# jthorborg/signalizer

Hardware: AMD Instinct MI355X
Metric: 32768-pt stereo STFT frames/sec (75% overlap); achieved HBM GB/s vs peak (higher is better)
Workload: dtype f32

## Files before the change

signalizer_amd/csrc/api.hip:

```cpp
#include <hip/hip_runtime.h>

#include <algorithm>
#include <chrono>
#include <cmath>
#include <atomic>
#include <cstdlib>
#include <cstring>
#include <deque>
#include <mutex>
#include <new>
#include <string>
#include <vector>

#include "runtime.hpp"
#include "trace.hpp"

namespace sgz {

thread_local std::string g_lastError;
#ifdef SGZ_SCHED_SWEEP
int g_schedule[7] = {-1, -1, -1, -1, -1, -1, -1};
#endif
#ifdef SGZ_DEBUG
uint32_t g_ablate = 0;
// ... 163 lines not shown
sgz_status resetResonator(Plan &p, hipStream_t stream)
{
    if (!isResonator(p) || !p.d_resState) return SGZ_OK;
    SGZ_HIP(hipMemsetAsync(p.d_resState, 0, size_t(p.C) * 2 * size_t(p.resV) * p.P * 2 * sizeof(float), stream));
    return SGZ_OK;
}

static sgz_status fillResParams(Plan &p, const float *d_planar, size_t chStride, long frames, float *d_mapped, uint32_t hopOverride, ResParams &r)
{
    r = ResParams{};
    r.planar = d_planar; r.chStride = chStride; r.frames = frames;
    r.hop = hopOverride ? hopOverride : p.cfg.hop; r.C = p.C; r.P = p.P; r.mode = p.cfg.channel_mode;
    r.V = p.resV; r.signals = p.stateChannels; r.sides = p.sides; r.firstContinues = true;
    r.coeff = reinterpret_cast<const float2 *>(p.d_resCoeff);
    r.cpow = reinterpret_cast<const float4 *>(p.d_resPow);
    r.cpowB = reinterpret_cast<const float2 *>(p.d_resPowB);
    r.cpowBLo = reinterpret_cast<const float2 *>(p.d_resPowBLo);
    r.matrixForm = p.optMatrixResonator;
    r.w1 = p.optMatrixResonator ? reinterpret_cast<const float2 *>(p.d_resW1) : nullptr;
    r.w2 = reinterpret_cast<const float2 *>(p.d_resW2);
    r.w1b = reinterpret_cast<const uint4 *>(p.d_resW1b);
    r.tilePow = reinterpret_cast<const float4 *>(p.d_resTile);
    r.gain = p.d_resGain;
    for (int v = 0; v < 9; ++v) r.weights[v] = p.resWeights[v];
    r.state = reinterpret_cast<float2 *>(p.d_resState);
    const size_t perFrame = size_t(p.C) * size_t(r.signals) * size_t(r.V) * p.P;
    sgz_status st = ensureCap(&p.d_resLocal, &p.resLocalCap, (size_t(frames) + size_t(kResSegments)) * perFrame * 2);
    if (st != SGZ_OK) return st;
    r.local = reinterpret_cast<float2 *>(p.d_resLocal);
    r.segEnd = r.local + size_t(frames) * perFrame;
    r.mapped = d_mapped;
    return SGZ_OK;
}

static sgz_status runResonator(Plan &p, const float *d_planar, size_t chStride, long frames, float *d_mapped, hipStream_t stream, uint32_t hopOverride = 0,
                               bool skipWindow = false)
{
    if (frames <= 0) return SGZ_OK;
    if (!d_mapped) return fail(SGZ_EUNSUPPORTED, "the resonator algorithm has no transform bins: ask for mapped values");
    if (hopOverride && frames != 1) return fail(SGZ_EINVAL, "a block advance of the resonators is one frame");
    if (!skipWindow && !hopOverride) {
        const size_t perFrame = size_t(p.C) * size_t(p.stateChannels) * size_t(p.resV) * p.P * 2 * sizeof(float);
        const long slab = p.optResonatorSlab ? long(p.optResonatorSlab) : long(std::max<size_t>(64, (size_t(256) << 20) / perFrame));
        if (frames > slab) {
            for (long f0 = 0; f0 < frames; f0 += slab) {
                const long nf = std::min(slab, frames - f0);
                const sgz_status st = runResonator(p, d_planar + size_t(f0) * p.cfg.hop, chStride, nf, d_mapped + size_t(f0) * p.C * p.sides * p.P, stream);
                if (st != SGZ_OK) return st;
            }
            return SGZ_OK;
        }
    }
    ResParams r;
    if (sgz_status st = fillResParams(p, d_planar, chStride, frames, d_mapped, hopOverride, r); st != SGZ_OK) return st;
    r.skipWindow = skipWindow;
    SGZ_HIP(launchResonator(r, stream));
    return SGZ_OK;
}

sgz_status checkResonatorShardBound(const Plan &p, long frames)
{
    const size_t perFrame = size_t(p.C) * size_t(p.stateChannels) * size_t(p.resV) * p.P * 2 * sizeof(float);
    const size_t bound = p.optResonatorShardBound ? size_t(p.optResonatorShardBound) : std::max<size_t>(64, (size_t(8) << 30) / std::max<size_t>(perFrame, 1));
    if (frames > 0 && size_t(frames) > bound)
        return fail(SGZ_EUNSUPPORTED, "sharded RSNT render: a rank's chunk of " + std::to_string(frames) + " frames holds " +
                                          std::to_string((size_t(frames) * perFrame) >> 20) + " MiB of per-frame resonator states between the two halves of the render, above the bound of " +
                                          std::to_string(bound) + " frames (SGZ_OPT_RESONATOR_SHARD_BOUND; default 8 GiB): use more ranks or a shorter buffer per call");
    return SGZ_OK;
}
sgz_status runResonatorFromRest(Plan &p, const float *d_planar, size_t chStride, long frames, float *d_mapped, hipStream_t stream)
{
    if (sgz_status st = checkResonatorShardBound(p, frames); st != SGZ_OK) return st;
    if (sgz_status st = resetResonator(p, stream); st != SGZ_OK) return st;
    return runResonator(p, d_planar, chStride, frames, d_mapped, stream, 0, true);
}
sgz_status runResonatorJoin(Plan &p, long frames, float *d_mapped, const float *d_allEnd, const long long *framesPerRank, uint32_t world, uint32_t rank,
                            float *d_carry, hipStream_t stream)
{
    if (frames <= 0) return SGZ_OK;
    ResParams r;
    if (sgz_status st = fillResParams(p, nullptr, 0, frames, d_mapped, 0, r); st != SGZ_OK) return st;
    const float2 *carry = nullptr;
    if (rank > 0) {
        SGZ_HIP(launchResonatorFold(r, reinterpret_cast<const float2 *>(d_allEnd), framesPerRank, world, rank, reinterpret_cast<float2 *>(d_carry), stream));
        carry = reinterpret_cast<const float2 *>(d_carry);
    }
    SGZ_HIP(launchResonatorCarry(r, carry, stream));
    return SGZ_OK;
}

sgz_status runResonatorAdvance(Plan &p, const float *d_planar, size_t chStride, uint32_t nsamples, float *d_mapped, hipStream_t stream)
{
    if (!isResonator(p)) return fail(SGZ_EINVAL, "not a resonator plan");
    if (nsamples == 0) return SGZ_OK;
    return runResonator(p, d_planar, chStride, 1, d_mapped, stream, nsamples);
}

sgz_status ensureSecondStream(Plan &p)
{
    if (!p.shardStream) { hipStream_t cs; SGZ_HIP(hipStreamCreateWithFlags(&cs, hipStreamNonBlocking)); p.shardStream = cs; }
    for (void *&e : p.shardEv)
        if (!e) { hipEvent_t ne; SGZ_HIP(hipEventCreateWithFlags(&ne, hipEventDisableTiming)); e = ne; }
    return SGZ_OK;
}

sgz_status runStft(Plan &p, const float *d_planar, size_t chStride, long frames, float *d_mapped,
                          float *d_binsOut, const float *d_binsIn, hipStream_t stream, unsigned long long *d_phaseClock, bool deferLate,
                          bool imageOnly)
{
    TraceRange range("sgz::runStft (K_A)");
    p.lateDeferred = nullptr; p.lateFrames = 0;
    if (isResonator(p)) {
        if (d_binsOut || d_binsIn) return fail(SGZ_EUNSUPPORTED, "the resonator algorithm has no transform bins");
        return runResonator(p, d_planar, chStride, frames, d_mapped, stream);
    }
    const bool phase = p.cfg.channel_mode == SGZ_CH_PHASE;
    StftParams prm = fillStftParams(p, d_planar, chStride, frames, d_mapped, d_binsOut, d_binsIn, d_phaseClock);
    const long tasks = frames * long(p.C);
    if (tasks <= 0) return SGZ_OK;
    if (tasks > 0x7fffffffL) return fail(SGZ_EINVAL, "too many (frame, pair) tasks for one launch");
    if (p.optChannelSplit && ((p.realMono && d_binsIn == nullptr) || p.realSplit)) {
        const size_t units = size_t(tasks) * 2;
        if (p.nyCap < units) {
            for (float **b : {&p.d_ny, &p.d_nyBest, &p.d_low}) if (*b) { (void)hipFree(*b); *b = nullptr; }
            p.nyCap = 0;
            SGZ_HIP(hipMalloc(reinterpret_cast<void **>(&p.d_nyBest), units * 64 * sizeof(float)));
            SGZ_HIP(hipMalloc(reinterpret_cast<void **>(&p.d_ny), units * sizeof(float)));
            SGZ_HIP(hipMalloc(reinterpret_cast<void **>(&p.d_low), units * kLowBins * sizeof(float)));
            p.nyCap = units;
        }
        RealParams rp{};
        rp.planar = d_planar; rp.chStride = chStride; rp.frames = frames;
        rp.hop = p.cfg.hop; rp.C = p.C; rp.P = p.P; rp.mode = p.cfg.channel_mode;
        rp.window = p.d_windowHalf;
        rp.winPhase = p.optFetchWindow ? nullptr : reinterpret_cast<const float4 *>(p.d_winPhase); rp.winP0 = 0.5f * p.winP0; rp.winP1 = 0.5f * p.winP1;
        rp.tw1 = reinterpret_cast<const float2 *>(p.d_twReal1);
        rp.tw2 = reinterpret_cast<const float2 *>(p.d_tw2);
        rp.twPost = reinterpret_cast<const float2 *>(p.d_twRealPost);
        rp.tw2Full = reinterpret_cast<const float4 *>(p.d_tw2Full);
        rp.recs = p.d_recsReal ? p.d_recsReal : p.d_recs; rp.recsFull = p.d_recs; rp.weights = p.d_weights;
        rp.chunkEnds = p.d_chunkEnds; rp.chunkReBase = p.d_chunkReBase; rp.chunkRec = p.d_chunkRec; rp.weights12 = p.d_weights12;
        rp.chunkSlots[0] = p.chunkSlots[0]; rp.chunkSlots[1] = p.chunkSlots[1];
        rp.low = p.d_low; rp.lowPixels = p.d_realLowPixels; rp.lowCount[0] = p.realLowCount[0]; rp.lowCount[1] = p.realLowCount[1];
        rp.invSize = p.scalars.invSize;
        rp.mapped = d_mapped; rp.binsOut = d_binsOut; rp.binsIn = d_binsIn;
        rp.ny = p.d_ny; rp.nyBest = p.d_nyBest;
        rp.fixFrom[0] = p.realFixFrom[0]; rp.fixFrom[1] = p.realFixFrom[1];
        if (deferLate && !p.realMono && d_mapped && !d_binsOut && p.realLowCount[0] + p.realLowCount[1] == 0) { rp.lateInNext = 1u; p.lateDeferred = d_mapped; p.lateFrames = frames; }
        rp.roundSize = uint32_t(numCUs()) * (p.N == 16384 ? 4u : p.N == 32768 ? 2u : 1u);
        rp.pipelined = p.optPipelined ? 1u : 0u;
        if (imageOnly && rp.lateInNext && p.optImageOnlySplit && p.realSplit && p.cfg.channel_mode == SGZ_CH_SEPARATE && p.N == 32768 &&
            rp.winPhase && p.C == 1) {
            const long room = long(rp.roundSize) - tasks;
            const long want = p.optImageOnlySplit >= 2 ? long(p.optImageOnlySplit) : room > 0 ? std::min<long>(8, std::max<long>(1, (tasks + room - 1) / room)) : 4;
            rp.nyFrames = uint32_t(std::min<long>(want, frames));
        }
        p.lastNyFrames = rp.nyFrames;
        if (rp.nyFrames && !rp.pipelined && tasks > long(rp.roundSize >> 1) && tasks < long(rp.roundSize)) {
            rp.mateAdjacent = SGZ_MATE_ADJACENT;
            const long nyUnits = long(p.C) * ((frames + long(rp.nyFrames) - 1) / long(rp.nyFrames));
            if (rp.nyFrames <= 3u && tasks + nyUnits <= long(rp.roundSize)) {
                rp.prioFirst = SGZ_PRIO_FIRST; rp.prioMate = SGZ_PRIO_MATE; rp.prioNy = SGZ_PRIO_NY; rp.prioScope = SGZ_PRIO_SCOPE;
            }
#ifdef SGZ_SCHED_SWEEP
            if (g_schedule[0] >= 0) rp.nyDelay = uint32_t(g_schedule[0]);
            if (g_schedule[1] >= 0) rp.mateDelay = uint32_t(g_schedule[1]);
            if (g_schedule[2] >= 0) rp.mateAdjacent = uint32_t(g_schedule[2]);
            if (g_schedule[3] >= 0) rp.prioFirst = uint32_t(g_schedule[3]) & 3u;
            if (g_schedule[4] >= 0) rp.prioMate = uint32_t(g_schedule[4]) & 3u;
            if (g_schedule[5] >= 0) rp.prioNy = uint32_t(g_schedule[5]) & 3u;
            if (g_schedule[6] >= 0) rp.prioScope = uint32_t(g_schedule[6]) & 3u;
#endif
        }
#ifdef SGZ_DEBUG
        rp.phaseClock = d_phaseClock; rp.clkUnit = g_ablate >> 16;
#endif
        SGZ_HIP(launchStftReal(rp, p.N, stream));
        return SGZ_OK;
    }
    if (p.halves && d_binsIn == nullptr) {
        const size_t perTask = size_t(p.N) + 1;
        long slab = long(std::max<size_t>(1, (size_t(32) << 20) / perTask));
        slab = std::max<long>(1, slab / long(p.C)) * long(p.C);
        slab = std::min<long>(slab, tasks);
        if (d_binsOut == nullptr && p.binsSlab < size_t(slab)) {
            if (p.d_halfBins) { (void)hipFree(p.d_halfBins); p.d_halfBins = nullptr; }
            SGZ_HIP(hipMalloc(reinterpret_cast<void **>(&p.d_halfBins), size_t(slab) * perTask * sizeof(float)));
            p.binsSlab = size_t(slab);
        }
        if (prm.nDcPixels) { sgz_status st = ensureDcWork(p, size_t(slab)); if (st != SGZ_OK) return st; prm.dcOut = reinterpret_cast<float2 *>(p.d_dcWork); }
        for (long t0 = 0; t0 < tasks; t0 += slab) {
            const long nt = std::min(slab, tasks - t0);
            float *bins = d_binsOut ? d_binsOut + size_t(t0) * perTask : p.d_halfBins;
            prm.taskBase = t0;
            prm.frames = nt / long(p.C);
            prm.binsOut = bins;
            prm.binsSplit = (d_binsOut == nullptr && p.sideMapOk && mapSidesFit(prm, p.N)) ? 1u : 0u;
            SGZ_HIP(launchStftHalves(prm, p.N, int(2 * nt), stream));
            if (d_mapped) {
                float *out = d_mapped + size_t(t0) * p.sides * p.P;
                if (prm.binsSplit) SGZ_HIP(launchMapSides(prm, p.N, bins, nt, out, stream));
                else SGZ_HIP(launchGenericMap(prm, p.N, bins, nt, out, stream));
                SGZ_HIP(launchComplexDcFix(prm, p.N, bins, prm.dcOut, nt, out, stream));
            }
        }
        return SGZ_OK;
    }
    if (!p.fused) {
        const size_t perTask = size_t(p.N) * 2;
        long slab = long(std::max<size_t>(1, (size_t(64) << 20) / perTask));
        slab = std::max<long>(1, slab / long(p.C)) * long(p.C);
        slab = std::min<long>(slab, tasks);
        if (p.workSlab < size_t(slab)) {
            for (float **b : {&p.d_work0, &p.d_work1, &p.d_binsWork}) if (*b) { (void)hipFree(*b); *b = nullptr; }
            SGZ_HIP(hipMalloc(reinterpret_cast<void **>(&p.d_work0), size_t(slab) * perTask * sizeof(float)));
            SGZ_HIP(hipMalloc(reinterpret_cast<void **>(&p.d_work1), size_t(slab) * perTask * sizeof(float)));
            SGZ_HIP(hipMalloc(reinterpret_cast<void **>(&p.d_binsWork), size_t(slab) * (size_t(p.N) + 1) * sizeof(float) * (phase ? 2 : 1)));
            p.workSlab = size_t(slab);
        }
        if (prm.nDcPixels) { sgz_status st = ensureDcWork(p, p.workSlab); if (st != SGZ_OK) return st; prm.dcOut = reinterpret_cast<float2 *>(p.d_dcWork); }
        PhaseTables ph{};
        if (phase) {
            ph.type = p.d_phaseType; ph.norm = p.d_phaseNorm; ph.normFinal = p.phaseNormFinal;
            ph.filtered = p.cfg.bin_interp != SGZ_INTERP_NONE;
            ph.fusedFft = p.phaseFusedFft ? 1u : 0u;
            ph.csfOut = reinterpret_cast<float2 *>(d_binsOut);
            ph.csfIn = reinterpret_cast<const float2 *>(d_binsIn);
        }
        SGZ_HIP(launchGeneric(prm, p.N, reinterpret_cast<const float2 *>(p.d_twN), reinterpret_cast<float2 *>(p.d_work0),
                              reinterpret_cast<float2 *>(p.d_work1), p.d_binsWork, long(p.workSlab), stream, phase ? &ph : nullptr,
                              p.sideMapOk && !phase));
        return SGZ_OK;
    }
    const int grid = int(tasks);
    SGZ_HIP(launchStftMap(prm, p.N, grid, stream));
    return SGZ_OK;
}

static sgz_status fillDecayParams(Plan &p, const float *d_mapped, long frames, uint8_t *d_rgba, float *d_lines, float *d_state,
                                  hipStream_t stream, DecayParams &prm)
{
    prm = DecayParams{};
    prm.mapped = d_mapped;
    prm.frames = frames;
    prm.P = p.P; prm.C = p.C; prm.sides = uint32_t(p.sides);
    prm.chunk = 8;
    prm.numChunks = uint32_t((frames + prm.chunk - 1) / prm.chunk);
    prm.slope = p.d_slope;
    prm.colourTables = p.d_colourTables;
    prm.sc = p.scalars;
    prm.state = d_state; prm.stateIn = d_state; prm.rgba = d_rgba; prm.lines = d_lines;
    prm.colourOnly = (!d_state && !d_lines && d_rgba) ? 1u : 0u;
    prm.magScale = p.cfg.channel_mode == SGZ_CH_PHASE ? 0.5f : 1.0f;
    if (d_state && frames > 1) {
        const size_t stateN = size_t(p.C) * SGZ_NUM_GRAPHS * p.P * 2;
        sgz_status st0 = ensureCap(&p.d_stateCopy, &p.stateCopyCap, stateN);
        if (st0 != SGZ_OK) return st0;
        if (prm.numChunks > 1 && p.cfg.channel_mode != SGZ_CH_PHASE) {
            prm.stateStash = p.d_stateCopy;
        } else {
            SGZ_HIP(hipMemcpyAsync(p.d_stateCopy, d_state, stateN * sizeof(float), hipMemcpyDeviceToDevice, stream));
            prm.stateIn = p.d_stateCopy;
        }
    }
    return SGZ_OK;
}

sgz_status runDecayColour(Plan &p, const float *d_mapped, long frames, uint8_t *d_rgba, float *d_lines,
                                 float *d_state, hipStream_t stream, bool magnitudeOnly)
{
    TraceRange range("sgz::runDecayColour (K_B)");
    float *pending = const_cast<float *>(p.lateDeferred);
    const long pendingFrames = p.lateFrames;
    p.lateDeferred = nullptr; p.lateFrames = 0;
    if (frames <= 0) return SGZ_OK;
    p.aggMapped = nullptr;
    DecayParams prm;
    sgz_status stp = fillDecayParams(p, d_mapped, frames, d_rgba, d_lines, d_state, stream, prm);
    if (stp != SGZ_OK) return stp;
    const bool noFused = !p.optFusedColour;
    prm.fusedPixels = p.optFusedPixels;
    const bool fullFused = !noFused && !magnitudeOnly && p.cfg.channel_mode != SGZ_CH_PHASE && prm.numChunks > 1 && decayFullFusedApplies(prm);
    if (pending) {
        if (d_mapped == pending && frames == pendingFrames && !noFused && p.cfg.channel_mode != SGZ_CH_PHASE && (decayColourFusedApplies(prm) || fullFused)) {
            prm.late = LateFix{p.d_ny, p.d_nyBest, p.realFixFrom[0], p.realFixFrom[1], p.P, p.scalars.invSize, 0u};
            prm.hasLate = 1u;
        } else {
            SGZ_HIP(launchRealLate(fillRealLate(p, pendingFrames, pending), p.N, stream));
        }
    }
    if (p.cfg.channel_mode == SGZ_CH_PHASE && !magnitudeOnly) {
        if (!noFused && decayColourFusedApplies(prm)) {
            SGZ_HIP(launchDecayColourFused(prm, stream));
            return SGZ_OK;
        }
        sgz_status stw = ensureCap(&p.d_phaseWork, &p.phaseWorkCap, size_t(frames) * p.C * p.P);
        if (stw != SGZ_OK) return stw;
        SGZ_HIP(launchDecayPhase(prm, p.d_phaseWork, stream));
        return SGZ_OK;
    }
    if (!noFused && decayColourFusedApplies(prm)) {
        SGZ_HIP(launchDecayColourFused(prm, stream));
        return SGZ_OK;
    }
    if (fullFused) {
        prm.stateStash = nullptr;
        SGZ_HIP(launchDecayFullFused(prm, stream));
// ... 898 lines not shown
```

signalizer_amd/csrc/spectrum_real.hip:

```cpp
#include <algorithm>

#include "real_common.hpp"

#ifdef SGZ_DEBUG
#define RCLK(slot)                                                                                                     \
    do {                                                                                                               \
        if (prm.phaseClock && (tid & 63) == 0 && unit == long(prm.clkUnit)) prm.phaseClock[16 * (tid >> 6) + (slot)] = __builtin_readcyclecounter(); \
    } while (0)
#define RTRACE(which)                                                                                                  \
    do {                                                                                                               \
        if (prm.phaseClock && prm.clkUnit == 0xffffu && tid == 0) {                                                    \
            unsigned long long *t = prm.phaseClock + 256 + 4 * unit;                                                   \
            t[which] = __builtin_amdgcn_s_memrealtime();                                                               \
            if (which == 0) { t[2] = __builtin_amdgcn_s_getreg(4 | (31 << 11)); t[3] = __builtin_amdgcn_s_getreg(20 | (31 << 11)) | (static_cast<unsigned long long>(blockIdx.x) << 32); } \
        }                                                                                                              \
    } while (0)
#else
#define RCLK(slot) do { } while (0)
#define RTRACE(which) do { } while (0)
#endif

namespace sgz {

template <int R1, int LR1, int BASE, int Q = 0>
__device__ __forceinline__ void e1WriteRun(uint32_t wa, const v2 (&c)[32])
{
    if constexpr (Q < R1) { ldsWrite64<(Q & 15) * 512 * 8>(wa + uint32_t(Q >> 4) * 65536u, c[BASE + brev(Q, LR1)]); e1WriteRun<R1, LR1, BASE, Q + 1>(wa, c); }
}

template <int R1, int LR1, int Q = 0>
__device__ __forceinline__ void e1WritePairRun(uint32_t wa, const v2 (&c)[32])
{
    if constexpr (Q < R1) { ldsWrite128<(Q & 15) * 512 * 8>(wa + uint32_t(Q >> 4) * 65536u, c[brev(Q, LR1)], c[R1 + brev(Q, LR1)]); e1WritePairRun<R1, LR1, Q + 1>(wa, c); }
}

template <int R, int R1, int U, int LR1, int u = 0>
__device__ __forceinline__ void pass1Columns(v2 (&c)[R])
{
    if constexpr (u < U) {
        ditPacked<LR1, u * R1>(c);
        pass1Columns<R, R1, U, LR1, u + 1>(c);
    }
}

constexpr float kRotA1Cm1 = -0x1.3bd3ccp-24f, kRotA1Sin = 0x1.921fb4p-12f;
constexpr float kRotA4Cm1 = -0x1.3bd3c8p-20f, kRotA4Sin = 0x1.921faap-10f;
__device__ __forceinline__ float4 rotatePhaseForward(const float4 ph, const float cm1, const float sn)
{
    const v2 pc = v2{ph.x, ph.y}, ps = v2{ph.z, ph.w};
    const v2 kc = v2{cm1, cm1}, ks = v2{sn, sn};
    const v2 c2 = __builtin_elementwise_fma(pc, kc, __builtin_elementwise_fma(ps, -ks, pc));
    const v2 s2 = __builtin_elementwise_fma(ps, kc, __builtin_elementwise_fma(pc, ks, ps));
    return float4{c2.x, c2.y, s2.x, s2.y};
}
__device__ __forceinline__ float2 rotateTwiddle(const float2 w, const float cm1, const float sn)
{
    const v2 v = v2{w.x, w.y}, sw = v2{w.y, w.x};
    const v2 r = __builtin_elementwise_fma(v, v2{cm1, cm1}, __builtin_elementwise_fma(sw, v2{sn, -sn}, v));
    return float2{r.x, r.y};
}

__device__ __forceinline__ void windowPairCos(v2 &lo, v2 &hi, const int a32, const v2 pc, const v2 ps, const v2 p0)
{
    v2 t = pc;
    if (a32 != 0) {
        const v2 k = v2{cos32(a32), sin32(a32)};
        v2 m;
        asm("v_pk_mul_f32 %0, %1, %2 op_sel:[0,1] op_sel_hi:[1,1]" : "=v"(m) : "v"(ps), "s"(k));
        asm("v_pk_fma_f32 %0, %1, %2, %3 op_sel:[0,0,0] op_sel_hi:[1,0,1] neg_lo:[0,0,1] neg_hi:[0,0,1]" : "=v"(t) : "v"(pc), "s"(k), "v"(m));
    }
    v2 wa, wb;
    asm("v_pk_add_f32 %0, %1, %2" : "=v"(wa) : "v"(t), "s"(p0));
    asm("v_pk_add_f32 %0, %1, %2 neg_lo:[1,0] neg_hi:[1,0]" : "=v"(wb) : "v"(t), "s"(p0));
    lo = lo * wa;
    hi = hi * wb;
}

template <int LR1, int MIX, typename P>
__device__ __forceinline__ void realMapSettle(const P &prm, float *lds, const int tid, const int side, const long task, const long self,
                                              const ChunkTables &tb, ChunkMap<(1 << (LR1 + 5))> &mapper, float *re, float *ce, float *spec)
{
    constexpr int R = 32, R1 = 1 << LR1, T = R1 * R, M = R1 * R * R, N = 2 * M;
    constexpr bool MONO = MIX == 1 || MIX == 3;
    const ChannelIndex at{N, side ? M : 0};
    [[maybe_unused]] const long unit = MONO ? task : self;
    if (prm.binsOut) {
        float *dst = prm.binsOut + size_t(task) * (N + 1) + (side ? M : 0);
        for (int i = tid; i <= M; i += T)
            if (MONO || i != (side ? 0 : M)) dst[i] = lds[chunkPos(i)];
    }
    if (!MONO && (prm.lowCount[0] + prm.lowCount[1]) && tid < kLowBins) prm.low[size_t(self) * kLowBins + tid] = lds[at(side ? N - tid : tid)];
    RCLK(8);
    mapper.run(tb, at, lds, re, ce, prm.invSize, tid);
    RCLK(9);
    RTRACE(1);
    if (MONO) {
        if (prm.mapped && prm.lowCount[0]) {
            float *out = prm.mapped + size_t(task) * prm.P;
            for (uint32_t i = tid; i < prm.lowCount[0]; i += T) {
                const uint32_t x = prm.lowPixels[i];
                out[x] = complexDcPixel(prm.recsFull[x], prm.weights, prm.invSize, N, prm.mode,
                                        [&](int k) { return k >= N ? 0.f : lds[chunkPos(k)]; },
                                        [&](int sl) { return make_float2(spec[2 * sl], spec[2 * sl + 1]); });
            }
        }
        return;
    }
}

[[maybe_unused]] __device__ __forceinline__ void setWavePriority(const uint32_t p)
{
    if (p != 0u) { if (p == 1u) __builtin_amdgcn_s_setprio(1); else if (p == 2u) __builtin_amdgcn_s_setprio(2); else __builtin_amdgcn_s_setprio(3); }
}

template <int LR1, bool PRIO>
__device__ __forceinline__ void nyquistUnit(const RealParams &prm, float *lds, const uint32_t light, const int tid)
{
    constexpr int LR = 5, R = 32, R1 = 1 << LR1, RR = R * R;
    static_assert(LR1 == 4, "the Nyquist workgroups mirror the two-columns-per-thread form (N = 32768)");
    [[maybe_unused]] const long unit = 2 * long(light) + 1;
    RTRACE(0);
#ifdef SGZ_IMAGE_PRIO
    if constexpr (PRIO) setWavePriority(prm.prioNy);
#endif
#ifdef SGZ_SCHED_SWEEP
    for (uint32_t k = 0; k < prm.nyDelay; ++k) __builtin_amdgcn_s_sleep(16);
#endif
    const uint32_t F = prm.nyFrames, perPair = uint32_t(prm.frames) / F + (uint32_t(prm.frames) % F != 0u);
    const uint32_t pair = light / perPair, f0 = (light - pair * perPair) * F;
    const uint32_t f1 = f0 + F < uint32_t(prm.frames) ? f0 + F : uint32_t(prm.frames);
    const float *X0 = prm.planar + size_t(2 * pair + 1) * prm.chStride;
    const uint32_t lane16 = uint32_t(tid) * 16u;
    const float4 ph[2] = {ldg(prm.winPhase, lane16 * 2u), ldg(prm.winPhase + 1, lane16 * 2u)};
    const v2 p0 = v2{prm.winP0, prm.winP0};
    v2 *lds2 = reinterpret_cast<v2 *>(lds);
    for (uint32_t f = f0; f < f1; ++f) {
        const float *X = X0 + size_t(f) * prm.hop;
#pragma unroll
        for (int u = 0; u < 2; ++u) {
            v2 c[R1];
#pragma unroll
            for (int j = 0; j < R1; ++j) c[j] = ldgPinned<v2>(X, uint32_t(RR * j) * 8u + 8u * u, lane16);
            const v2 pc = v2{ph[u].x, ph[u].y}, ps = v2{ph[u].z, ph[u].w};
#pragma unroll
            for (int j = 0; j < R1 / 2; ++j) windowPairCos(c[j], c[j + R1 / 2], j * (32 / R1), pc, ps, p0);
            ditPacked<LR1, 0>(c);
            lds2[2 * tid + u] = c[0];
        }
        __syncthreads();
        if (tid < R) {
            v2 s[R];
#pragma unroll
            for (int h = 0; h < R; ++h) s[h] = lds2[tid + R * h];
            ditPacked<LR, 0>(s);
            lds2[RR + tid] = s[0];
        }
        __syncthreads();
        if (tid == 0) {
            v2 s[R];
#pragma unroll
            for (int r = 0; r < R; ++r) s[r] = lds2[RR + r];
            const float4 *tab = prm.tw2Full;
#pragma unroll
            for (int i = 0; i < R / 4; ++i) {
                const float4 wa = tab[i], wb = tab[i + R / 4];
                if (i == 0) bflyPackedFusedTw<true>(s[0], s[R / 2], v2{1.f, 0.f}, v2{wb.x, wb.y});
                else bflyPackedFusedTw<false>(s[2 * i], s[2 * i + R / 2], v2{wa.x, wa.y}, v2{wb.x, wb.y});
                bflyPackedFusedTw<false>(s[2 * i + 1], s[2 * i + 1 + R / 2], v2{wa.z, wa.w}, v2{wb.z, wb.w});
            }
            ditPacked<LR, 0, R, 2>(s);
            prm.ny[((size_t(f) * prm.C + pair) << 1) | 1u] = 2.f * (s[0].x - s[0].y);
        }
    }
    RTRACE(1);
}

template <int LR1, bool WCOS, int MIX = 0, bool PRIO = false>
__global__ void __launch_bounds__(1 << (LR1 + 5), 4) stftRealKernel(const RealParams launchPrm)
{
    constexpr int LR = 5, R = 32, R1 = 1 << LR1, T = R1 * R, RR = R * R, M = R1 * RR, N = 2 * M, U = R / R1;
    constexpr bool MONO = MIX == 1 || MIX == 3;
    constexpr bool SIDE0 = MIX == 4;
    constexpr bool mixed = MIX == 2 || MIX == 3;
    constexpr int PADSTRIDE = chunkPos(T);
    constexpr int ROW = R + 2, TILE = R * ROW;
    constexpr int XFLOATS = realXFloats(M);
    static_assert((T / R) * TILE <= XFLOATS, "the exchange-2 tiles end below the twiddle table");
    constexpr int TAB = (XFLOATS + 3) & ~3;
    extern __shared__ __attribute__((aligned(16))) float lds[];
    const int tid0 = threadIdx.x;

    constexpr bool WALK = LR1 == 5 && MIX == 0 && WCOS;
    const uint32_t heavyUnits = SIDE0 ? uint32_t(launchPrm.frames) * launchPrm.C : gridDim.x;
    if constexpr (SIDE0) {
        if (blockIdx.x >= heavyUnits) { nyquistUnit<LR1, PRIO>(launchPrm, lds, blockIdx.x - heavyUnits, opaque(tid0)); return; }
    }
    const uint32_t totalUnits = WALK ? uint32_t(launchPrm.frames) * launchPrm.C * 2u : heavyUnits;
    uint32_t walkIndex = blockIdx.x;
    UnitId uid = unitOfIndex<MONO || SIDE0>(launchPrm, walkIndex, totalUnits, SIDE0 && launchPrm.mateAdjacent != 0u);
    [[maybe_unused]] bool firstUnit = true;
    [[maybe_unused]] uint32_t prioEarly = 0u, prioLate = 0u, prioEnds = 0u;
    if constexpr (LR1 == 4) {
        const uint32_t cus = launchPrm.roundSize >> 1;
#ifndef SGZ_STAGGER
#define SGZ_STAGGER 5
#endif
        if (cus && !launchPrm.pipelined && gridDim.x >= 2u * cus && blockIdx.x >= cus && blockIdx.x < 2u * cus) {
#pragma unroll
            for (int k = 0; k < SGZ_STAGGER; ++k) __builtin_amdgcn_s_sleep(32);
        }
#ifdef SGZ_SCHED_SWEEP
        else if (SIDE0 && blockIdx.x >= cus) {
            for (uint32_t k = 0; k < launchPrm.mateDelay; ++k) __builtin_amdgcn_s_sleep(16);
        }
#endif
#ifndef SGZ_NO_PRIO
        if (cus && !launchPrm.pipelined && gridDim.x > 2u * cus && gridDim.x <= 3u * cus) {
#else
        if (false) {
#endif
            const uint32_t generation = blockIdx.x / cus;
            if (generation == 0u) __builtin_amdgcn_s_setprio(2); else if (generation == 1u) __builtin_amdgcn_s_setprio(1); else __builtin_amdgcn_s_setprio(3);
        }
#ifdef SGZ_IMAGE_PRIO
        if constexpr (PRIO) {
#ifdef SGZ_SCHED_SWEEP
            const uint32_t rolePrio = blockIdx.x >= cus ? launchPrm.prioMate : blockIdx.x + cus < heavyUnits ? launchPrm.prioFirst : 0u;
            const uint32_t scope = launchPrm.prioScope;
#else
            const uint32_t rolePrio = blockIdx.x >= cus ? (launchPrm.prioMate ? uint32_t(SGZ_PRIO_MATE) : 0u)
                                                        : blockIdx.x + cus < heavyUnits ? (launchPrm.prioFirst ? uint32_t(SGZ_PRIO_FIRST) : 0u) : 0u;
            constexpr uint32_t scope = SGZ_PRIO_SCOPE;
#endif
            prioEarly = (scope == 0u || scope == 3u) ? rolePrio : 0u;
            prioLate = (scope == 1u || scope == 2u) ? rolePrio : 0u;
            prioEnds = (scope & 1u) ? rolePrio : 0u;
            prioEarly = __builtin_amdgcn_readfirstlane(prioEarly); prioLate = __builtin_amdgcn_readfirstlane(prioLate); prioEnds = __builtin_amdgcn_readfirstlane(prioEnds);
        }
#endif
    }
    constexpr bool PAIRED = U == 2;
    constexpr int COLSTEP = PAIRED ? 1 : T, COLLANE = PAIRED ? 2 : 1;
    constexpr bool FRONT = LR1 >= 4 && !mixed && WCOS;
#ifdef SGZ_DIET
    constexpr bool DIET = PAIRED && FRONT && LR1 == 4;
#else
    constexpr bool DIET = false;
#endif
    [[maybe_unused]] float4 phase[U];
    [[maybe_unused]] float2 twA[U], twB[U];
    [[maybe_unused]] float4 tw2piece, tw2tail;
    v2 c[R];
    for (;;) {
    typename ParamsOf<WALK>::T &prm = *ParamsOf<WALK>::get(launchPrm);
    auto samplesOf = [&](const UnitId &u) {
        const int firstCh = MONO ? (prm.mode == SGZ_CH_RIGHT ? 1 : 0) : (mixed ? 0 : u.side);
        return prm.planar + size_t(2 * u.pair + firstCh) * prm.chStride + size_t(u.frame) * prm.hop;
    };
    auto elemOf = [&](int e) { const int u = e / R1, j = e % R1; return (PAIRED ? u : T * u) + RR * j; };
    auto requestSamples = [&](const float *X, const int tid, auto partTag) {
        constexpr int part = decltype(partTag)::value;
        const uint32_t lane8 = uint32_t(tid) * (PAIRED ? 16u : 8u);
        if constexpr (PAIRED) {
            typedef float v4 __attribute__((ext_vector_type(4)));
#pragma unroll
            for (int j = 0; j < R1; ++j) { const v4 xv = ldgPinned<v4>(X, uint32_t(RR * j) * 8u, lane8); c[j] = v2{xv.x, xv.y}; c[R1 + j] = v2{xv.z, xv.w}; }
        } else {
#pragma unroll
            for (int i = 0; i < R; ++i)
                if (part == 0 || ((i >> 3) & 1) == part - 1) c[i] = ldgPinned<v2>(X, uint32_t(elemOf(i)) * 8u, lane8);
        }
    };
    auto requestTables = [&](const int tid) {
        if constexpr (FRONT) {
            if constexpr (WALK) tw2piece = prm.tw2Full[tid < kTw2Floats / 4 ? tid : 0];
#pragma unroll
            for (int u = 0; u < (DIET ? 1 : U); ++u) {
                if (WCOS) phase[u] = ldg(prm.winPhase + COLSTEP * u, uint32_t(tid) * 16u * COLLANE);
                twA[u] = ldg(prm.tw1 + (COLSTEP * u), uint32_t(tid) * 8u * COLLANE);
                twB[u] = ldg(prm.tw1 + (COLSTEP * u + 3 * RR), uint32_t(tid) * 8u * COLLANE);
            }
            if constexpr (!WALK) { if (tid < kTw2Floats / 4) tw2piece = prm.tw2Full[tid]; }
            if (T < kTw2Floats / 4 && tid < kTw2Floats / 4 - T) tw2tail = prm.tw2Full[T + tid];
        }
    };
    if constexpr (WALK) {
        if (firstUnit) requestSamples(samplesOf(uid), tid0, std::integral_constant<int, 1>{});
        firstUnit = false;
    }
    const int tid = WALK ? opaque(tid0) : tid0;
    const int slot = tid >> 6, half = (tid >> 5) & 1, l = tid & 31, group = tid >> 5;
    const int q1 = half ? (slot == 0 ? R1 / 2 : R1 - slot) : slot;
    const int ix = half ? R - 1 - l : l;
    const uint32_t lane8 = uint32_t(tid) * (PAIRED ? 16u : 8u);
    [[maybe_unused]] const long unit = MONO ? long(uid.task) : long(uid.self);
    const int side = uid.side, pair = uid.pair;
    const long task = uid.task, frame = uid.frame, self = uid.self;

    const uint32_t maxSlots = prm.chunkSlots[0] > prm.chunkSlots[1] ? prm.chunkSlots[0] : prm.chunkSlots[1];
    const ChunkTables tb{prm.chunkEnds + side * T, prm.chunkReBase + side * T,
                         reinterpret_cast<const uint2 *>(prm.chunkRec) + size_t(side) * prm.P, prm.recs + size_t(side) * prm.P, prm.weights12,
                         prm.mapped ? prm.mapped + (size_t(task) * (MONO ? 1 : 2) + side) * prm.P : nullptr,
                         MONO ? nullptr : prm.nyBest + size_t(self) * 64, int(prm.fixFrom[side]), int(prm.P), side != 0,
#ifdef SGZ_DEBUG
                         (prm.phaseClock && unit == long(prm.clkUnit)) ? prm.phaseClock : nullptr};
#else
                         nullptr};
#endif
    const ChannelIndex at{N, side ? M : 0};
    float *re = lds + XFLOATS, *ce = re + maxSlots + 1;
    const int SCRATCH = XFLOATS + int(realExtraFloats(maxSlots, T, LR1 >= 4));
    float *spec = lds + SCRATCH + 2 * R;
    ChunkMap<T> mapper;

    RCLK(0);
    RTRACE(0);
    if constexpr (LR1 >= 4 && !FRONT) {
        for (int i = tid; i < kTw2Floats / 4; i += T) reinterpret_cast<float4 *>(lds + TAB)[i] = prm.tw2Full[i];
    }
    {
        const float *X = samplesOf(uid);
        if constexpr (WALK) {
            requestTables(tid);
            __builtin_amdgcn_sched_barrier(0);
            requestSamples(X, tid, std::integral_constant<int, 2>{});
            __builtin_amdgcn_sched_barrier(0);
            if (tid < kTw2Floats / 4) reinterpret_cast<float4 *>(lds + TAB)[tid] = tw2piece;
        } else {
            requestSamples(X, tid, std::integral_constant<int, 0>{});
            requestTables(tid);
        }
        if constexpr (FRONT) __builtin_amdgcn_sched_barrier(0);
#ifdef SGZ_IMAGE_PRIO
        if constexpr (PRIO) setWavePriority(prioEarly);
#endif
        if (mixed) {
            const float *Y = X + prm.chStride;
            const float sgn = (MONO ? prm.mode == SGZ_CH_SIDE : side == 1) ? -1.f : 1.f;
            constexpr int YB = (LR1 == 5 || (PAIRED && !WCOS)) ? 4 : 8;
#pragma unroll
            for (int b0 = 0; b0 < R; b0 += YB) {
                float2 y[YB];
#pragma unroll
                for (int i = 0; i < YB; ++i) y[i] = ldg(reinterpret_cast<const float2 *>(Y) + elemOf(b0 + i), lane8);
#pragma unroll
                for (int i = 0; i < YB; ++i) c[b0 + i] = v2{c[b0 + i].x + sgn * y[i].x, c[b0 + i].y + sgn * y[i].y};
                __builtin_amdgcn_sched_barrier(0);
            }
        }
        if (WCOS) {
            const v2 p0 = v2{prm.winP0, prm.winP0};
#pragma unroll
            for (int u = 0; u < U; ++u) {
                const float4 ph = (DIET && u == 1) ? rotatePhaseForward(phase[0], kRotA1Cm1, kRotA1Sin)
                                  : FRONT ? phase[u] : ldg(prm.winPhase + COLSTEP * u, uint32_t(tid) * 16u * COLLANE);
                const v2 pc = v2{ph.x, ph.y}, ps = v2{ph.z, ph.w};
#pragma unroll
                for (int j = 0; j < R1 / 2; ++j) {
                    constexpr int S32 = 32 / R1;
                    const int a32 = j * S32;
                    const int i = u * R1 + j, i2 = i + R1 / 2;
                    if constexpr (LR1 == 3) {
                        const float cj = cos32(a32), sj = sin32(a32);
                        const float te = a32 == 0 ? ph.x : ph.x * cj - ph.z * sj, to = a32 == 0 ? ph.y : ph.y * cj - ph.w * sj;
                        c[i] = v2{c[i].x * (prm.winP0 + te), c[i].y * (prm.winP0 + to)};
                        c[i2] = v2{c[i2].x * (prm.winP0 - te), c[i2].y * (prm.winP0 - to)};
                        continue;
                    }
                    windowPairCos(c[i], c[i2], a32, pc, ps, p0);
                }
            }
        } else {
            constexpr int B = LR1 >= 4 ? 4 : 8;
            float2 wa[B], wb[B];
#pragma unroll
            for (int i = 0; i < B; ++i) wa[i] = ldg(reinterpret_cast<const float2 *>(prm.window) + elemOf(i), lane8);
#pragma unroll
            for (int b0 = 0; b0 < R; b0 += 2 * B) {
#pragma unroll
                for (int i = 0; i < B; ++i) wb[i] = ldg(reinterpret_cast<const float2 *>(prm.window) + elemOf(b0 + B + i), lane8);
                __builtin_amdgcn_sched_barrier(0);
#pragma unroll
                for (int i = 0; i < B; ++i) { c[b0 + i] = v2{c[b0 + i].x * wa[i].x, c[b0 + i].y * wa[i].y}; asm volatile("" : "+v"(c[b0 + i])); }
                if (b0 + 2 * B < R) {
#pragma unroll
                    for (int i = 0; i < B; ++i) wa[i] = ldg(reinterpret_cast<const float2 *>(prm.window) + elemOf(b0 + 2 * B + i), lane8);
                }
                __builtin_amdgcn_sched_barrier(0);
#pragma unroll
                for (int i = 0; i < B; ++i) { c[b0 + B + i] = v2{c[b0 + B + i].x * wb[i].x, c[b0 + B + i].y * wb[i].y}; asm volatile("" : "+v"(c[b0 + B + i])); }
            }
        }
    }
    if (mixed) {
#pragma unroll
        for (int i = 0; i < R; ++i) c[i] = v2{c[i].x * 0.5f, c[i].y * 0.5f};
    }
    __builtin_amdgcn_sched_barrier(0);
    RCLK(13);
    pass1Columns<R, R1, U, LR1>(c);
#ifdef SGZ_IMAGE_PRIO
    if constexpr (PRIO) setWavePriority(prioLate);
#endif
#pragma unroll
    for (int u = 0; u < U; ++u) {
        constexpr int NB = R1 / 4 - 1;
        float2 a[3], b[NB];
        auto sq = [](float2 w) { return float2{w.x * w.x - w.y * w.y, 2.f * w.x * w.y}; };
        auto mul = [](float2 p, float2 q) { return float2{p.x * q.x - p.y * q.y, p.x * q.y + p.y * q.x}; };
        if (DIET && u == 1) {
            a[0] = rotateTwiddle(twA[0], kRotA1Cm1, kRotA1Sin);
            if (NB > 0) b[0] = rotateTwiddle(twB[0], kRotA4Cm1, kRotA4Sin);
        } else {
            a[0] = FRONT ? twA[u] : ldg(prm.tw1 + (COLSTEP * u), uint32_t(tid) * 8u * COLLANE);
            if (NB > 0) b[0] = FRONT ? twB[u] : ldg(prm.tw1 + (COLSTEP * u + 3 * RR), uint32_t(tid) * 8u * COLLANE);
        }
        a[1] = sq(a[0]); a[2] = mul(a[1], a[0]);
#pragma unroll
        for (int i = 1; i < NB; ++i) b[i] = (i & 1) ? sq(b[i / 2]) : mul(b[i - 1], b[0]);
#pragma unroll
        for (int q = 1; q < R1; ++q) {
            const int qa = q >> 2, qb = q & 3;
            v2 w;
            if (qa == 0) w = v2{a[qb - 1].x, a[qb - 1].y};
            else if (qb == 0) w = v2{b[qa - 1].x, b[qa - 1].y};
            else w = cmul(v2{b[qa - 1].x, b[qa - 1].y}, v2{a[qb - 1].x, a[qb - 1].y});
            const int i = u * R1 + brev(q, LR1);
            c[i] = cmul(c[i], w);
        }
    }
    RCLK(1);
    {
        v2 *lds2 = reinterpret_cast<v2 *>(lds);
        auto writeRound = [&](int r) {
            if constexpr (PAIRED) {
                if ((tid >> 8) == r) e1WritePairRun<R1, LR1>(ldsAddress(lds2 + ((2 * tid) & 511)), c);
                return;
            }
#pragma unroll
            for (int u = 0; u < U; ++u) {
                const int col = COLLANE * tid + COLSTEP * u;
                if ((col >> 9) == r) {
#ifndef SGZ_E1_PAIRED_WRITES
                    const uint32_t wa = ldsAddress(lds2 + (col & 511));
                    if (u == 0) e1WriteRun<R1, LR1, 0>(wa, c);
                    else if (u == 1) e1WriteRun<R1, LR1, (U > 1 ? R1 : 0)>(wa, c);
                    else if (u == 2) e1WriteRun<R1, LR1, (U > 2 ? 2 * R1 : 0)>(wa, c);
                    else e1WriteRun<R1, LR1, (U > 3 ? 3 * R1 : 0)>(wa, c);
#else
// ... 235 lines not shown
template <int LR1>
__global__ void __launch_bounds__(1 << (LR1 + 5)) realMapFromBinsKernel(const RealParams prm)
{
    constexpr int R = 32, R1 = 1 << LR1, T = R1 * R, M = R1 * R * R, N = 2 * M;
    constexpr int XFLOATS = realXFloats(M);
    extern __shared__ __attribute__((aligned(16))) float lds[];
    const int tid = threadIdx.x;
    const long unit = blockIdx.x;
    const int side = int(unit & 1);
    const long task = unit >> 1;
    const long self = (task << 1) | side;
    const uint32_t maxSlots = prm.chunkSlots[0] > prm.chunkSlots[1] ? prm.chunkSlots[0] : prm.chunkSlots[1];
    const ChunkTables tb{prm.chunkEnds + side * T, prm.chunkReBase + side * T,
                         reinterpret_cast<const uint2 *>(prm.chunkRec) + size_t(side) * prm.P, prm.recs + size_t(side) * prm.P, prm.weights12,
                         prm.mapped ? prm.mapped + (size_t(task) * 2 + side) * prm.P : nullptr, prm.nyBest + size_t(self) * 64, int(prm.fixFrom[side]), int(prm.P), side != 0, nullptr};
    float *re = lds + XFLOATS, *ce = re + maxSlots + 1;
    ChunkMap<T> mapper;
    mapper.prefetch(tb, tid);
    const float *src = prm.binsIn + size_t(task) * (N + 1) + (side ? M : 0);
    for (int i = tid; i <= M; i += T) lds[chunkPos(i)] = (i == (side ? 0 : M)) ? 0.f : src[i];
    *reinterpret_cast<float2 *>(lds + chunkPos(32 * tid) + 32) = float2{0.f, 0.f};
    if (tid < 16) lds[chunkPos(M) + 1 + tid] = 0.f;
    if (tid == 0) prm.ny[self] = src[side ? 0 : M];
    __syncthreads();
    realMapSettle<LR1, 0>(prm, lds, tid, side, task, self, tb, mapper, re, ce, lds);
}

__host__ __device__ LateFix lateFixOf(const RealParams &prm)
{
    return LateFix{prm.ny, prm.nyBest, prm.fixFrom[0], prm.fixFrom[1], prm.P, prm.invSize, prm.binsIn ? 1u : 0u};
}
__global__ void __launch_bounds__(256) realLateKernel(const RealParams prm, const int N, const uint32_t nTop)
{
#pragma clang fp contract(off)
    const long tasks = prm.frames * long(prm.C);
    const long item = long(blockIdx.x) * 256 + threadIdx.x;
    const long tops = tasks * 2 * nTop;
    const uint32_t nLow = prm.lowCount[0] + prm.lowCount[1];
    if (item < tops) {
        const long task = item / (2 * nTop);
        const int s = int((item / nTop) & 1);
        const uint32_t j = uint32_t(item % nTop);
        const LateFix lf = lateFixOf(prm);
        const uint32_t x = lf.fixFrom(s) + j;
        const bool top = x < prm.P && prm.mapped;
        float *px = prm.mapped + size_t(2 * task + s) * prm.P + (top ? x : 0u);
        const float own = top ? *px : 0.f;
        const float best = top ? lateBestSquare(lf, task, s, x) : 0.f;
        const float vM = lateNyquistBin(lf, task);
        if (s == 0 && j == 0 && prm.binsOut) prm.binsOut[size_t(task) * (N + 1) + N / 2] = vM;
        if (top) {
            const float v = lateNyquistPixel(lf, vM, best, own);
            if (v != own || !(own == own)) *px = v;
        }
    } else if (item < tops + tasks * nLow && prm.mapped) {
        const long task = (item - tops) / nLow;
        const uint32_t n = uint32_t((item - tops) % nLow);
        const int s = n < prm.lowCount[0] ? 0 : 1;
        const uint32_t x = prm.lowPixels[n];
        const PixelRec rec = prm.recsFull[size_t(s) * prm.P + x];
        const float *lowL = prm.low + size_t(2 * task) * kLowBins, *lowR = lowL + kLowBins;
        float acc = 0.f;
        int k = rec.a;
        for (int i = 0; i < rec.b; ++i) {
            const float v = k < kLowBins ? lowL[k] : lowR[N - k];
            acc = acc + v * prm.weights[rec.c + i];
            k = (k == N) ? 0 : k + 1;
        }
        prm.mapped[(size_t(2 * task + s)) * prm.P + x] = finishPixel<5>(prm.invSize * acc);
    }
}
hipError_t launchRealLate(const RealParams &prm, uint32_t N, hipStream_t stream)
{
    const long tasks = prm.frames * long(prm.C);
    if (tasks <= 0) return hipSuccess;
    uint32_t nTop = 1;
    for (int s = 0; s < 2; ++s) nTop = std::max(nTop, std::min(64u, prm.P - std::min(prm.P, prm.fixFrom[s])));
    const long items = tasks * 2 * nTop + tasks * long(prm.lowCount[0] + prm.lowCount[1]);
    hipLaunchKernelGGL(realLateKernel, dim3(unsigned((items + 255) / 256)), dim3(256), 0, stream, prm, int(N), nTop);
    return hipGetLastError();
}

__global__ void __launch_bounds__(256) finishPixelKernel(const float *x, float *y, size_t n)
{
    const size_t i = size_t(blockIdx.x) * blockDim.x + threadIdx.x;
    if (i < n) y[i] = finishPixel<5>(x[i]);
}
hipError_t launchFinishPixel(const float *x, float *y, size_t n, hipStream_t stream)
{
    if (n == 0) return hipSuccess;
    hipLaunchKernelGGL(finishPixelKernel, dim3(unsigned((n + 255) / 256)), dim3(256), 0, stream, x, y, n);
    return hipGetLastError();
}

hipError_t launchStftReal(const RealParams &prm, uint32_t N, hipStream_t stream)
{
    const bool mono = prm.mode != SGZ_CH_SEPARATE && prm.mode != SGZ_CH_MIDSIDE;
    const bool side0 = prm.nyFrames && N == 32768 && prm.mode == SGZ_CH_SEPARATE && prm.winPhase && prm.lateInNext && prm.mapped && !prm.binsOut &&
                       !prm.binsIn && prm.lowCount[0] + prm.lowCount[1] == 0;
    const long tasks = prm.frames * long(prm.C);
    const long units = side0 ? tasks + long(prm.C) * ((prm.frames + prm.nyFrames - 1) / prm.nyFrames) : tasks * (mono ? 1 : 2);
    if (units <= 0) return hipSuccess;
    const uint32_t M = N / 2, T = M / 32;
    const uint32_t maxSlots = std::max(prm.chunkSlots[0], prm.chunkSlots[1]);
    const size_t ldsBytes = (size_t(realXFloats(int(M))) + realExtraFloats(maxSlots, T, N >= 32768) + 64 + (mono ? 2 * kSpecBins : 0)) * 4;
    static size_t granted[29][64] = {};
    const bool wcos = prm.winPhase != nullptr;
    if (prm.binsIn) {
        if (mono) return hipErrorNotSupported;
        auto inject = [&](auto kern, int slot, unsigned threads) -> hipError_t {
            if (hipError_t e = grantLds(reinterpret_cast<const void *>(kern), ldsBytes, granted[slot]); e != hipSuccess) return e;
            hipLaunchKernelGGL(kern, dim3(unsigned(units)), dim3(threads), ldsBytes, stream, prm);
            return launchRealLate(prm, N, stream);
        };
        if (N == 32768) return inject(&realMapFromBinsKernel<4>, 24, 512);
        if (N == 16384) return inject(&realMapFromBinsKernel<3>, 25, 256);
        if (N == 65536) return inject(&realMapFromBinsKernel<5>, 26, 1024);
        return hipErrorNotSupported;
    }
    auto go = [&](auto kern, int slot, unsigned threads, size_t limit) -> hipError_t {
        if (ldsBytes > limit) return hipErrorInvalidValue;
        if (hipError_t e = grantLds(reinterpret_cast<const void *>(kern), ldsBytes, granted[slot]); e != hipSuccess) return e;
        const bool walk = N == 65536 && !mono && prm.mode == SGZ_CH_SEPARATE && wcos && prm.roundSize;
        hipLaunchKernelGGL(kern, dim3(unsigned(walk ? std::min<long>(units, long(prm.roundSize)) : units)), dim3(threads), ldsBytes, stream, prm);
        if (!mono && !prm.lateInNext) return launchRealLate(prm, N, stream);
        return hipSuccess;
    };
    hipError_t e;
    if (mono && (prm.mode == SGZ_CH_MERGE || prm.mode == SGZ_CH_SIDE)) {
        if (N == 32768) e = wcos ? go(&stftRealKernel<4, true, 3>, 18, 512, 80 * 1024) : go(&stftRealKernel<4, false, 3>, 19, 512, 80 * 1024);
        else if (N == 16384) e = wcos ? go(&stftRealKernel<3, true, 3>, 20, 256, 40 * 1024) : go(&stftRealKernel<3, false, 3>, 21, 256, 40 * 1024);
        else if (N == 65536) e = wcos ? go(&stftRealKernel<5, true, 3>, 22, 1024, 160 * 1024) : go(&stftRealKernel<5, false, 3>, 23, 1024, 160 * 1024);
        else return hipErrorNotSupported;
        if (e != hipSuccess) return e;
        return hipGetLastError();
    }
    if (mono) {
        if (N == 32768) e = wcos ? go(&stftRealKernel<4, true, 1>, 6, 512, 80 * 1024) : go(&stftRealKernel<4, false, 1>, 7, 512, 80 * 1024);
        else if (N == 16384) e = wcos ? go(&stftRealKernel<3, true, 1>, 8, 256, 40 * 1024) : go(&stftRealKernel<3, false, 1>, 9, 256, 40 * 1024);
        else if (N == 65536) e = wcos ? go(&stftRealKernel<5, true, 1>, 10, 1024, 160 * 1024) : go(&stftRealKernel<5, false, 1>, 11, 1024, 160 * 1024);
        else return hipErrorNotSupported;
        if (e != hipSuccess) return e;
        return hipGetLastError();
    }
    if (prm.mode == SGZ_CH_MIDSIDE) {
        if (N == 32768) e = wcos ? go(&stftRealKernel<4, true, 2>, 12, 512, 80 * 1024) : go(&stftRealKernel<4, false, 2>, 13, 512, 80 * 1024);
        else if (N == 16384) e = wcos ? go(&stftRealKernel<3, true, 2>, 14, 256, 40 * 1024) : go(&stftRealKernel<3, false, 2>, 15, 256, 40 * 1024);
        else if (N == 65536) e = wcos ? go(&stftRealKernel<5, true, 2>, 16, 1024, 160 * 1024) : go(&stftRealKernel<5, false, 2>, 17, 1024, 160 * 1024);
        else return hipErrorNotSupported;
        if (e != hipSuccess) return e;
        return hipGetLastError();
    }
#ifdef SGZ_IMAGE_PRIO
    if (side0 && (prm.prioFirst | prm.prioMate | prm.prioNy)) e = go(&stftRealKernel<4, true, 4, true>, 28, 512, 80 * 1024);
    else
#endif
    if (side0) e = go(&stftRealKernel<4, true, 4>, 27, 512, 80 * 1024);
    else if (N == 32768) e = wcos ? go(&stftRealKernel<4, true>, 0, 512, 80 * 1024) : go(&stftRealKernel<4, false>, 1, 512, 80 * 1024);
    else if (N == 16384) e = wcos ? go(&stftRealKernel<3, true>, 4, 256, 40 * 1024) : go(&stftRealKernel<3, false>, 5, 256, 40 * 1024);
    else if (N == 65536) e = wcos ? go(&stftRealKernel<5, true>, 2, 1024, 160 * 1024) : go(&stftRealKernel<5, false>, 3, 1024, 160 * 1024);
    else return hipErrorNotSupported;
    if (e != hipSuccess) return e;
    return hipGetLastError();
}

}
```

Measured before the change: 14.51 million.

## Reuse overlapping hop rows in Nyquist units across consecutive frames

Nyquist workgroups handling several consecutive frames now keep the loaded input rows in registers and shift them by the hop. With 75% overlap only the newly exposed rows are fetched per frame, which cuts redundant global loads. Registers are parked in LDS during the reduction trees to ease register pressure. The heuristic for frames per Nyquist unit is retuned, and side is fixed to zero for SIDE0 kernels. The trade-off is more register and LDS traffic and an extra kernel-variant selection path.

```diff
diff --git a/signalizer_amd/csrc/api.hip b/signalizer_amd/csrc/api.hip
--- a/signalizer_amd/csrc/api.hip
+++ b/signalizer_amd/csrc/api.hip
@@ -339,7 +339,8 @@
         if (imageOnly && rp.lateInNext && p.optImageOnlySplit && p.realSplit && p.cfg.channel_mode == SGZ_CH_SEPARATE && p.N == 32768 &&
             rp.winPhase && p.C == 1) {
             const long room = long(rp.roundSize) - tasks;
-            const long want = p.optImageOnlySplit >= 2 ? long(p.optImageOnlySplit) : room > 0 ? std::min<long>(8, std::max<long>(1, (tasks + room - 1) / room)) : 4;
+            const long fit = room > 0 ? std::max<long>(1, (tasks + room - 1) / room) : 0;
+            const long want = p.optImageOnlySplit >= 2 ? long(p.optImageOnlySplit) : room <= 0 ? 4 : fit <= 6 ? fit : 3;
             rp.nyFrames = uint32_t(std::min<long>(want, frames));
         }
         p.lastNyFrames = rp.nyFrames;
diff --git a/signalizer_amd/csrc/spectrum_real.hip b/signalizer_amd/csrc/spectrum_real.hip
--- a/signalizer_amd/csrc/spectrum_real.hip
+++ b/signalizer_amd/csrc/spectrum_real.hip
@@ -113,7 +113,8 @@
     if (p != 0u) { if (p == 1u) __builtin_amdgcn_s_setprio(1); else if (p == 2u) __builtin_amdgcn_s_setprio(2); else __builtin_amdgcn_s_setprio(3); }
 }
 
-template <int LR1, bool PRIO>
+constexpr uint32_t kNyHopRows = 4;
+template <int LR1, bool PRIO, bool SHARE>
 __device__ __forceinline__ void nyquistUnit(const RealParams &prm, float *lds, const uint32_t light, const int tid)
 {
     constexpr int LR = 5, R = 32, R1 = 1 << LR1, RR = R * R;
@@ -134,20 +135,14 @@
     const float4 ph[2] = {ldg(prm.winPhase, lane16 * 2u), ldg(prm.winPhase + 1, lane16 * 2u)};
     const v2 p0 = v2{prm.winP0, prm.winP0};
     v2 *lds2 = reinterpret_cast<v2 *>(lds);
-    for (uint32_t f = f0; f < f1; ++f) {
-        const float *X = X0 + size_t(f) * prm.hop;
-#pragma unroll
-        for (int u = 0; u < 2; ++u) {
-            v2 c[R1];
-#pragma unroll
-            for (int j = 0; j < R1; ++j) c[j] = ldgPinned<v2>(X, uint32_t(RR * j) * 8u + 8u * u, lane16);
-            const v2 pc = v2{ph[u].x, ph[u].y}, ps = v2{ph[u].z, ph[u].w};
-#pragma unroll
-            for (int j = 0; j < R1 / 2; ++j) windowPairCos(c[j], c[j + R1 / 2], j * (32 / R1), pc, ps, p0);
-            ditPacked<LR1, 0>(c);
-            lds2[2 * tid + u] = c[0];
-        }
-        __syncthreads();
+    auto columnSum = [&](v2 (&c)[R1], const int u) {
+        const v2 pc = v2{ph[u].x, ph[u].y}, ps = v2{ph[u].z, ph[u].w};
+#pragma unroll
+        for (int j = 0; j < R1 / 2; ++j) windowPairCos(c[j], c[j + R1 / 2], j * (32 / R1), pc, ps, p0);
+        ditPacked<LR1, 0>(c);
+        lds2[2 * tid + u] = c[0];
+    };
+    auto tree2 = [&]() {
         if (tid < R) {
             v2 s[R];
 #pragma unroll
@@ -155,7 +150,8 @@
             ditPacked<LR, 0>(s);
             lds2[RR + tid] = s[0];
         }
-        __syncthreads();
+    };
+    auto tree3 = [&](const uint32_t f) {
         if (tid == 0) {
             v2 s[R];
 #pragma unroll
@@ -171,6 +167,63 @@
             ditPacked<LR, 0, R, 2>(s);
             prm.ny[((size_t(f) * prm.C + pair) << 1) | 1u] = 2.f * (s[0].x - s[0].y);
         }
+    };
+    constexpr uint32_t HOPROWS = kNyHopRows;
+    if (SHARE && f1 - f0 > 1u && prm.hop == HOPROWS * 2u * uint32_t(RR)) {
+        typedef float v4 __attribute__((ext_vector_type(4)));
+        v4 raw[R1];
+        {
+            const float *X = X0 + size_t(f0) * prm.hop;
+#pragma unroll
+            for (int j = 0; j < R1; ++j) raw[j] = ldgPinned<v4>(X, uint32_t(RR * j) * 8u, lane16);
+        }
+        for (uint32_t f = f0; f < f1; ++f) {
+#pragma unroll
+            for (int u = 0; u < 2; ++u) {
+                v2 c[R1];
+#pragma unroll
+                for (int j = 0; j < R1; ++j) c[j] = u ? v2{raw[j].z, raw[j].w} : v2{raw[j].x, raw[j].y};
+                columnSum(c, u);
+            }
+            if (f + 1u < f1) {
+                const float *X = X0 + size_t(f + 1u) * prm.hop;
+#pragma unroll
+                for (int j = 0; j < R1 - int(HOPROWS); ++j) raw[j] = raw[j + int(HOPROWS)];
+#pragma unroll
+                for (int j = R1 - int(HOPROWS); j < R1; ++j) raw[j] = ldgPinned<v4>(X, uint32_t(RR * j) * 8u, lane16);
+            }
+            constexpr int PARK = R1 - int(HOPROWS);
+            v4 *park = reinterpret_cast<v4 *>(lds + 4 * RR) + (tid & 63);
+            if (__builtin_amdgcn_readfirstlane(tid) < 64) {
+                __syncthreads();
+#pragma unroll
+                for (int j = 0; j < PARK; ++j) park[64 * j] = raw[j];
+                tree2();
+                __syncthreads();
+                tree3(f);
+#pragma unroll
+                for (int j = 0; j < PARK; ++j) raw[j] = park[64 * j];
+            } else {
+                __syncthreads();
+                __syncthreads();
+            }
+        }
+        RTRACE(1);
+        return;
+    }
+    for (uint32_t f = f0; f < f1; ++f) {
+        const float *X = X0 + size_t(f) * prm.hop;
+#pragma unroll
+        for (int u = 0; u < 2; ++u) {
+            v2 c[R1];
+#pragma unroll
+            for (int j = 0; j < R1; ++j) c[j] = ldgPinned<v2>(X, uint32_t(RR * j) * 8u + 8u * u, lane16);
+            columnSum(c, u);
+        }
+        __syncthreads();
+        tree2();
+        __syncthreads();
+        tree3(f);
     }
     RTRACE(1);
 }
@@ -193,7 +246,7 @@
     constexpr bool WALK = LR1 == 5 && MIX == 0 && WCOS;
     const uint32_t heavyUnits = SIDE0 ? uint32_t(launchPrm.frames) * launchPrm.C : gridDim.x;
     if constexpr (SIDE0) {
-        if (blockIdx.x >= heavyUnits) { nyquistUnit<LR1, PRIO>(launchPrm, lds, blockIdx.x - heavyUnits, opaque(tid0)); return; }
+        if (blockIdx.x >= heavyUnits) { nyquistUnit<LR1, PRIO, PRIO>(launchPrm, lds, blockIdx.x - heavyUnits, opaque(tid0)); return; }
     }
     const uint32_t totalUnits = WALK ? uint32_t(launchPrm.frames) * launchPrm.C * 2u : heavyUnits;
     uint32_t walkIndex = blockIdx.x;
@@ -294,7 +347,7 @@
     const int ix = half ? R - 1 - l : l;
     const uint32_t lane8 = uint32_t(tid) * (PAIRED ? 16u : 8u);
     [[maybe_unused]] const long unit = MONO ? long(uid.task) : long(uid.self);
-    const int side = uid.side, pair = uid.pair;
+    const int side = SIDE0 ? 0 : uid.side, pair = uid.pair;
     const long task = uid.task, frame = uid.frame, self = uid.self;
 
     const uint32_t maxSlots = prm.chunkSlots[0] > prm.chunkSlots[1] ? prm.chunkSlots[0] : prm.chunkSlots[1];
@@ -836,7 +889,8 @@
         return hipGetLastError();
     }
 #ifdef SGZ_IMAGE_PRIO
-    if (side0 && (prm.prioFirst | prm.prioMate | prm.prioNy)) e = go(&stftRealKernel<4, true, 4, true>, 28, 512, 80 * 1024);
+    if (side0 && ((prm.prioFirst | prm.prioMate | prm.prioNy) || (prm.nyFrames > 1u && prm.frames > 1 && prm.hop == kNyHopRows * 2048u)))
+        e = go(&stftRealKernel<4, true, 4, true>, 28, 512, 80 * 1024);
     else
 #endif
     if (side0) e = go(&stftRealKernel<4, true, 4>, 27, 512, 80 * 1024);
```

Measured after the change: 14.67 million, median of 6. 1.01x the previous value.
